# dan64/vs-deoldify

Measured on AMD Instinct MI355X. Metric: colorized frames/sec/GPU @1080p (DeOldify stable rf=35); CIEDE2000 vs ref, higher is better.
Workload: dtype f16

## Files before the change

include/havc_mi355.h:

```cpp
#ifndef HAVC_MI355_H
#define HAVC_MI355_H

#include <stddef.h>
#include <stdint.h>

#ifdef __cplusplus
extern "C" {
#endif

#define HAVC_OK 0
#define HAVC_E_INVALID (-1)
#define HAVC_E_OOM (-2)
#define HAVC_E_HIP (-3)
#define HAVC_E_NODEVICE (-4)
#define HAVC_E_RANGE (-5)

typedef struct havc_ctx havc_ctx;
typedef struct havc_weights havc_weights;
typedef struct havc_net havc_net;

enum havc_op_type {
    HAVC_OP_CONV = 1,
    HAVC_OP_MAXPOOL = 2,
    HAVC_OP_BLUR_RESIZE = 3,
// ... 359 lines not shown
int havc_colormnet_rgb_to_lab(havc_ctx* ctx, const uint8_t* rgb, float* lab, int width, int height);
int havc_colormnet_lab_to_rgb(havc_ctx* ctx, const float* l_plane, const float* ab, uint8_t* rgb, int width, int height);

int havc_cmn_frame_in(havc_ctx* ctx, const uint8_t* rgb, float* lab, float* img, int width, int height, int padded_w, int padded_h, int pad_left,
                      int pad_top);
int havc_cmn_frame_out(havc_ctx* ctx, const float* l_plane, const float* ab_padded, uint8_t* rgb, int width, int height, int padded_w, int padded_h,
                       int pad_left, int pad_top);
int havc_memory_read_banked(havc_ctx* ctx, const float* mk, const float* ms, const float* qk, const float* qe, const float* mv, float* out,
                            float* use_count, float* life_count, int usage_from, int CK, int CV, int N, int64_t pitch, int HW, int top_k);
int havc_memory_read_reserve(havc_ctx* ctx, int N_max, int HW, int top_k);
int havc_cmn_short_term(havc_ctx* ctx, havc_net* net, int first_op, int n_ops, int agg_buf, int short_buf, const float* q, const float* k, const float* v,
                        const float* rel_w, const float* rel_b, float* agg, float* attn, float* short_out, int C, int CV, int H, int W, int max_dis);
int havc_cmn_join_add(havc_ctx* ctx, float* readout, const float* short_out, int64_t n);
int havc_cmn_side_mark(havc_ctx* ctx);
int havc_cmn_side_begin(havc_ctx* ctx);
int havc_cmn_side_end(havc_ctx* ctx);
int havc_cmn_side_wait(havc_ctx* ctx, int apply_usage);
int havc_cmn_value_in(havc_ctx* ctx, const float* image, const float* planes, float* value_in, int64_t pixels);
int havc_dev_copy_2d(havc_ctx* ctx, void* d_dst, size_t dst_pitch, const void* d_src, size_t src_pitch, size_t width_bytes, size_t rows);
int havc_net_bind_many(havc_net* net, int count, const int32_t* bufs, void* const* device_ptrs);
int havc_net_enqueue_slices(havc_net* net, int count, const int32_t* first_op, const int32_t* n_ops, const int32_t* batch);
int havc_debug_stream_jitter(int seed, int max_us);
const char* havc_build_stamp(void);

int havc_tag_timing_enable(havc_ctx* ctx, int tag, int enable);
int havc_tag_timing_read(havc_ctx* ctx, double* avg_ms, int64_t* launches);

#ifdef __cplusplus
}
#endif
#endif
```

vsdeoldify_amd/_native.py:

```python
import ctypes as C
import os

import numpy as np

_HERE = os.path.dirname(os.path.abspath(__file__))
LIB_PATH = os.environ.get("HAVC_MI355_LIB") or os.path.join(_HERE, "lib", "libhavc_mi355.so")

HAVC_OK, HAVC_E_INVALID, HAVC_E_OOM, HAVC_E_HIP, HAVC_E_NODEVICE, HAVC_E_RANGE = 0, -1, -2, -3, -4, -5
RESIZE_SPLINE64, RESIZE_SPLINE36 = 0, 1

OP_CONV, OP_MAXPOOL, OP_BLUR_RESIZE, OP_AFFINE, OP_ATTENTION, OP_PREP_RGB8, OP_COPY_CH = 1, 2, 3, 4, 5, 6, 7
OP_SUBSAMPLE2, OP_PROJ2, OP_BILINEAR2, OP_PREP_LAB_L = 8, 9, 10, 11
OP_DWCONV7, OP_LAYERNORM, OP_MHA, OP_PIXSHUF4_BLUR, OP_PREP_DDCOLOR, OP_DWCONV7_LN = 12, 13, 14, 15, 16, 17
OP_FOLD_QUERIES, OP_SHUF4_BLUR_AB = 18, 19
OP_EW, OP_DWCONV, OP_CHAN_ATTN, OP_MHA64, OP_CBAM, OP_GRU, OP_PLANAR_IN, OP_PLANAR_OUT, OP_CMN_DECODER_IN = 20, 21, 22, 23, 24, 25, 26, 27, 28
OP_SRCREF_ATTN, OP_TSTACK, OP_ELU, OP_PREP_REMASTER, OP_REMASTER_OUT = 29, 30, 31, 32, 33
EW_SRC_BCAST, EW_RES, EW_RES_BCAST, EW_RELU, EW_DUAL = 1, 2, 4, 8, 16
F_RELU_PRE, F_AFFINE, F_RESIDUAL, F_RELU_POST = 0x1, 0x2, 0x4, 0x8
F_OUT_PIXSHUF, F_OUT_TRANSPOSED, F_OUT_RGB8, F_LEAKY, F_FUSE_RGB8, F_PS_BLUR = 0x10, 0x20, 0x40, 0x80, 0x100, 0x200
F_GELU, F_W_FROM_BUF = 0x400, 0x800
F_FUSE_PROJ = 0x2000
F_PRECISE = 0x4000


# ... 214 lines not shown
    ("havc_batcher_create", _I, [_P, _P, _P, _F, _I, _I, _I, C.POINTER(_P)]),
    ("havc_batcher_create_frames", _I, [_P, _I, _P, _I, _I, _I, _I, C.POINTER(_P)]),
    ("havc_batcher_submit", _I, [_P, _P, _P]),
    ("havc_batcher_stats", _I, [_P, C.POINTER(C.c_int64), C.POINTER(C.c_int64)]),
    ("havc_batcher_free", None, [_P]),
    ("havc_cmn_frame_in", _I, [_P, _P, _P, _P, _I, _I, _I, _I, _I, _I]),
    ("havc_cmn_frame_out", _I, [_P, _P, _P, _P, _I, _I, _I, _I, _I, _I]),
    ("havc_memory_read_banked", _I, [_P, _P, _P, _P, _P, _P, _P, _P, _P, _I, _I, _I, _I, C.c_int64, _I, _I]),
    ("havc_memory_read_reserve", _I, [_P, _I, _I, _I]),
    ("havc_cmn_short_term", _I, [_P, _P, _I, _I, _I, _I, _P, _P, _P, _P, _P, _P, _P, _P, _I, _I, _I, _I, _I]),
    ("havc_cmn_join_add", _I, [_P, _P, _P, C.c_int64]),
    ("havc_cmn_side_mark", _I, [_P]),
    ("havc_cmn_side_begin", _I, [_P]),
    ("havc_ctx_set_stream_priority", _I, [_P, _I]),
    ("havc_ctx_set_stream_cus", _I, [_P, _I]),
    ("havc_cmn_side_end", _I, [_P]),
    ("havc_cmn_side_wait", _I, [_P, _I]),
    ("havc_cmn_value_in", _I, [_P, _P, _P, _P, C.c_int64]),
    ("havc_dev_copy_2d", _I, [_P, _P, _SZ, _P, _SZ, _SZ, _SZ]),
    ("havc_net_bind_many", _I, [_P, _I, _P, _P]),
    ("havc_net_enqueue_slices", _I, [_P, _I, _P, _P, _P]),
    ("havc_debug_stream_jitter", _I, [_I, _I]),
    ("havc_build_stamp", C.c_char_p, []),
    ("havc_tag_timing_enable", _I, [_P, _I, _I]),
    ("havc_tag_timing_read", _I, [_P, C.POINTER(C.c_double), C.POINTER(C.c_int64)]),
]


def _preload_torch_hip_runtime():
    if os.environ.get("HAVC_NO_TORCH_HIP_PRELOAD"):
        return
    try:
        import importlib.util
        spec = importlib.util.find_spec("torch")
        if spec is not None and spec.submodule_search_locations:
            p = os.path.join(list(spec.submodule_search_locations)[0], "lib", "libamdhip64.so")
            if os.path.exists(p):
                C.CDLL(p, mode=C.RTLD_GLOBAL)
    except Exception:
        pass


def load():
    global _lib
    if _lib is not None:
        return _lib
# ... 280 lines not shown
```

vsdeoldify_amd/csrc/conv_common.h:

```cpp
#pragma once
#include "kernels.h"
#include "../../include/havc_mi355.h"

typedef _Float16 half8 __attribute__((ext_vector_type(8)));
typedef _Float16 half4 __attribute__((ext_vector_type(4)));
typedef float float4v __attribute__((ext_vector_type(4)));

__device__ __forceinline__ float gelu_erf(float v) {
    const float L2E = 1.44269504088896341f;
    const float v2 = fminf(v * v, 36.0f);
    float p = fmaf(-1.72152684e-05f * -L2E, v2, -5.10199108e-04f * -L2E);
    p = fmaf(p, v2, 7.34616312e-02f * -L2E);
    p = fmaf(p, v2, 1.59538024f * -L2E);
    const float e = __builtin_amdgcn_exp2f(p * v);
    return v * __builtin_amdgcn_rcpf(1.0f + e);
}

__device__ __forceinline__ int64_t out_pixel(const ConvArgs& p, int m, int HoWo) {
    if (p.oss == 1) return m;
    const int b = m / HoWo, rem = m - b * HoWo, ho = rem / p.Wo, wo = rem - ho * p.Wo;
    return ((int64_t)(b * p.Ho * p.oss + ho * p.oss + p.ooy)) * (p.Wo * p.oss) + wo * p.oss + p.oox;
}

__device__ __forceinline__ void split_hl(float v, half_t& hi, half_t& lo) {
    hi = (half_t)v;
    lo = (half_t)((v - (float)hi) * 2048.f);
}
__device__ __forceinline__ float join_hl(half_t hi, half_t lo) { return (float)hi + (float)lo * (1.f / 2048.f); }

__device__ __forceinline__ void epilogue_frag_precise(const ConvArgs& p, const float4v acc, int m, int n, int HoWo) {
    const bool leaky = p.flags & HAVC_F_LEAKY;
    float v[4];
#pragma unroll
    for (int r = 0; r < 4; ++r) v[r] = acc[r] * p.pscale;
    if (p.bias) {
        const float4 bv = *reinterpret_cast<const float4*>(p.bias + n);
        v[0] += bv.x; v[1] += bv.y; v[2] += bv.z; v[3] += bv.w;
    }
    if (p.flags & HAVC_F_OUT_RGB8) {
        if (n == 0) {
            uint8_t* y = reinterpret_cast<uint8_t*>(p.y) + (int64_t)m * 3;
#pragma unroll
            for (int r = 0; r < 3; ++r) {
// ... 149 lines not shown
```

vsdeoldify_amd/csrc/conv_pipe_epilogue.inc:

```
    if (ABL == 5 || ABL == 9 || ABL == 10) {
        float t = 0.f;
#pragma unroll
        for (int mi = 0; mi < FM; ++mi)
#pragma unroll
            for (int ni = 0; ni < FN; ++ni) t += acc[ni][mi][0] + acc[ni][mi][1] + acc[ni][mi][2] + acc[ni][mi][3];
        if (t == 123.456f) reinterpret_cast<half_t*>(p.y)[0] = (half_t)t;
        return;
    }
    constexpr bool PRECISE = (ABL == 30);
    const bool lds_epi = !PRECISE && !(eflags & (HAVC_F_OUT_TRANSPOSED | HAVC_F_OUT_RGB8)) &&
                         (!(eflags & HAVC_F_OUT_PIXSHUF) || (p.Co & 63) == 0);
    bool fused_done = false;
    if (PRECISE && EXTRA && has_extra && (eflags & HAVC_F_FUSE_RGB8)) {
        fused_done = true;
        const bool leaky = eflags & HAVC_F_LEAKY;
        const int rlo = p.res_cpitch >> 1;
        auto fold = [&](const float4v a4, int m, int n, float d[3]) {
            if (n >= p.Npad) return;
            float v[4];
            const float4 bv = p.bias ? *reinterpret_cast<const float4*>(p.bias + n) : make_float4(0.f, 0.f, 0.f, 0.f);
            const float bb[4] = {bv.x, bv.y, bv.z, bv.w};
#pragma unroll
            for (int r = 0; r < 4; ++r) {
                v[r] = a4[r] * p.pscale + bb[r];
// ... 384 lines not shown
#pragma unroll
                for (int w = 0; w < 5; ++w) t += part[(w * BM + pl) * 3 + jo];
                float sg = 1.f / (1.f + __expf(-t));
                sg = sg * (p.f1 - p.f0) + p.f0;
                sg = sg * p.istd[jo] + p.mean[jo];
                sg = fminf(fmaxf(sg, 0.f), 1.f);
                y[jo] = (uint8_t)(int)(sg * 255.f);
            }
        }
    } else if (!EXTRA && (eflags & HAVC_F_FUSE_PROJ) && WM == 2 && WN == 4 && FM == 8) {
        fused_done = true;
        const bool leaky = eflags & HAVC_F_LEAKY;
        const int nw0 = n0 + wn * 64, cw0 = wn * 64;
        float4 bvs[FN];
#pragma unroll
        for (int ni = 0; ni < FN; ++ni)
            bvs[ni] = p.bias ? *reinterpret_cast<const float4*>(p.bias + nw0 + ni * 16 + lg * 4) : make_float4(0.f, 0.f, 0.f, 0.f);
        float4v facc[FM];
        int fb_prev = -1;
        half4 wa[FN];
#pragma unroll
        for (int mi = 0; mi < FM; ++mi) {
            const int mf = gm(wm * (FM * 16) + mi * 16);
            const int fb = mf < p.M ? mf / HoWo : 0;
            if (fb != fb_prev) {
                fb_prev = fb;
#pragma unroll
                for (int ni = 0; ni < FN; ++ni) {
                    wa[ni] = half4{0, 0, 0, 0};
                    if (lr < 2) {
                        const float4 w4 = *reinterpret_cast<const float4*>(p.fuse_w + ((size_t)fb * 2 + lr) * 256 + cw0 + ni * 16 + lg * 4);
                        wa[ni] = half4{(half_t)w4.x, (half_t)w4.y, (half_t)w4.z, (half_t)w4.w};
                    }
                }
            }
            facc[mi] = float4v{0.f, 0.f, 0.f, 0.f};
#pragma unroll
            for (int ni = 0; ni < FN; ++ni) {
                const float bb[4] = {bvs[ni].x, bvs[ni].y, bvs[ni].z, bvs[ni].w};
                half4 o;
#pragma unroll
                for (int r = 0; r < 4; ++r) {
                    float v = acc[ni][mi][r] + bb[r];
                    if (eflags & HAVC_F_RELU_PRE) v = v > 0.f ? v : (leaky ? v * p.f2 : 0.f);
                    o[r] = (half_t)v;
                }
                facc[mi] = __builtin_amdgcn_mfma_f32_16x16x16f16(wa[ni], o, facc[mi], 0, 0, 0);
// ... 38 lines not shown
        char* img = smem + wave * (FM * 2048);
#pragma unroll
        for (int ni = 0; ni < FN; ++ni) {
            const float4 bv = bvA[ni], sc = scA[ni], sh = shA[ni];
            const float bb[4] = {bv.x, bv.y, bv.z, bv.w}, ss[4] = {sc.x, sc.y, sc.z, sc.w}, hh[4] = {sh.x, sh.y, sh.z, sh.w};
#pragma unroll
            for (int mi = 0; mi < FM; ++mi) {
                half4 o;
#pragma unroll
                for (int r = 0; r < 4; ++r) {
                    float v = acc[ni][mi][r] + bb[r];
                    if (eflags & HAVC_F_RELU_PRE) v = v > 0.f ? v : (leaky ? v * p.f2 : 0.f);
                    if (eflags & HAVC_F_GELU) v = gelu_erf(v);
                    if (eflags & HAVC_F_AFFINE) v = v * ss[r] + hh[r];
                    o[r] = (half_t)v;
                }
                const int slot = (ni * 2 + (lg >> 1)) ^ (lp & 7);
                *reinterpret_cast<half4*>(img + mi * 2048 + lp * 128 + slot * 16 + (lg & 1) * 8) = o;
            }
        }
        if ((eflags & HAVC_F_PS_BLUR) && WM == 2 && WN == 4 && FM == 8) {
            __syncthreads();
            const int tile = m0 / BM, tt = p.tiles_y * p.tiles_x;
            const int b = tile / tt, t = tile - b * tt, ty = t / p.tiles_x, tx = t - ty * p.tiles_x;
            const int h0 = ty * 15 - 1, w0 = tx * 15 - 1, H2 = 2 * p.Ho, W2 = 2 * p.Wo;
            half_t* y = reinterpret_cast<half_t*>(p.y) + p.y_coff + (n0 >> 2);
            if (tid < 30 * 2 * 8 && (!p.cstore || (n0 >> 2) + (tid & 7) * 8 < p.cstore)) {
                const int ch = tid & 7, xh = (tid >> 3) & 1, Yl = tid >> 4;
                const int Y = 2 * (h0 + 1) + Yl;
                const int ay0 = max(Y - 1, 0);
                auto ld = [&](int ay, int ax) -> half8 {
                    const int dy = (ay >> 1) - h0, dx = (ax >> 1) - w0, q = (ay & 1) * 2 + (ax & 1);
                    return *reinterpret_cast<const half8*>(smem + ((dy >> 3) * WN + q) * (FM * 2048) + (dy & 7) * 2048 + dx * 128 + ((ch ^ (dx & 7)) << 4));
                };
                if (Y < H2) {
                    const int X0 = 2 * (w0 + 1) + xh * 15;
                    float l0[8], l1[8];
                    {
                        const int axl = max(X0 - 1, 0);
                        const half8 a = ld(ay0, axl), c = ld(Y, axl);
#pragma unroll
                        for (int e = 0; e < 8; ++e) { l0[e] = (float)a[e]; l1[e] = (float)c[e]; }
                    }
                    half_t* yrow = y + ((int64_t)(b * H2 + Y) * W2) * p.y_cpitch + ch * 8;
#pragma unroll 5
                    for (int k = 0; k < 15; ++k) {
                        const int X = X0 + k;
// ... 25 lines not shown
        if (eflags & HAVC_F_RESIDUAL) {
#pragma unroll
            for (int mi = 0; mi < FM; ++mi)
#pragma unroll
                for (int hp = 0; hp < 2; ++hp) {
                    const int m = gm(wm * (FM * 16) + PF(mi) * 16 + (lane >> 3) + hp * 8);
                    rres[mi][hp] = half8{0, 0, 0, 0, 0, 0, 0, 0};
                    if (do_res && m < p.M) rres[mi][hp] = *reinterpret_cast<const half8*>(p.res + opix(m) * p.res_cpitch + p.res_coff + n);
                }
        }
#pragma unroll
        for (int mi = 0; mi < FM; ++mi) {
#pragma unroll
            for (int hp = 0; hp < 2; ++hp) {
                const int px = (lane >> 3) + hp * 8;
                const int m = gm(wm * (FM * 16) + PF(mi) * 16 + px);
                const half8 v = *reinterpret_cast<const half8*>(img + mi * 2048 + px * 128 + ((ch ^ (px & 7)) << 4));
                if (m >= p.M) continue;
                half_t* y = reinterpret_cast<half_t*>(p.y);
                int64_t off;
                if (eflags & HAVC_F_OUT_PIXSHUF) {
                    const int q = n / p.Co, cc = n - q * p.Co;
                    if (q >= 4) continue;
                    const int b = m / HoWo, rem = m - b * HoWo, ho = rem / p.Wo, wo = rem - ho * p.Wo;
                    off = ((int64_t)(b * 2 * p.Ho + 2 * ho + (q >> 1)) * (2 * p.Wo) + 2 * wo + (q & 1)) * p.y_cpitch + p.y_coff + cc;
                } else {
                    if (n >= p.Co) continue;
                    off = opix(m) * p.y_cpitch + p.y_coff + n;
                }
                half8 o = v;
                if (eflags & (HAVC_F_RESIDUAL | HAVC_F_RELU_POST)) {
#pragma unroll
                    for (int e = 0; e < 8; ++e) {
                        float f = (float)v[e];
                        if (eflags & HAVC_F_RESIDUAL) f += (float)rres[mi][hp][e];
                        if (eflags & HAVC_F_RELU_POST) f = f > 0.f ? f : (leaky ? f * p.f2 : 0.f);
                        o[e] = (half_t)f;
                    }
                }
                if (ABL == 12) { if (o[0] == (half_t)123.f && o[1] == (half_t)77.f) *reinterpret_cast<half8*>(y + off) = o; }
                else if (ABL == 14) *reinterpret_cast<half8*>(y + (off & 0xFFFF8)) = o;
                else if (eflags & HAVC_F_NT_STORE) __builtin_nontemporal_store(o, reinterpret_cast<half8*>(y + off));
                else *reinterpret_cast<half8*>(y + off) = o;
            }
        }
    }
    if (EXTRA && has_extra && !(fused_done)) {
#pragma unroll
// ... 6 lines not shown
```

vsdeoldify_amd/csrc/conv_pipe_kernel.inc:

```
namespace {

constexpr int FN = 4;
constexpr unsigned OOB = 0xF0000000u;

template <int WM, int WN, int FM, int EXTRA>
struct Geo {
    static constexpr int NW = WM * WN;
    static constexpr int BM = WM * FM * 16, BN = WN * 64;
    static constexpr int A_IT = BM / 8 / NW, B_IT = BN / 8 / NW;
    static constexpr int NS = 2 * FM;
    static constexpr int PIECES = A_IT + B_IT;
    static constexpr int ROWS = BM + BN + 16 * EXTRA;
    static constexpr int STAGE_BYTES = ROWS * 128;
    static constexpr int LDS_BYTES = 2 * STAGE_BYTES;
    static_assert(BM % (8 * NW) == 0 && BN % (8 * NW) == 0 && NW % 2 == 0, "pieces must divide over an even number of waves");
    static_assert(FM >= FN, "second-half weight fragments are prefetched during the first FM steps");
    static_assert(FM % 2 == 0, "the 4-slot pixel-fragment ring wraps cleanly only when a stage has a multiple of 4 steps");
    static_assert(!EXTRA || (WM == 2 && WN == 4 && FM == 8), "extra columns: 256x256 tile only");
    static_assert(NW * FM * 2048 <= LDS_BYTES, "LDS epilogue image");
};

typedef __attribute__((address_space(3))) void* lds_ptr_t;

__device__ __forceinline__ void dma16(__amdgpu_buffer_rsrc_t rsrc, char* lds_wave_base, unsigned voff, unsigned soff) {
// ... 60 lines not shown
    const int kt0 = SK > 1 ? ((KT * part / SK) & ~1) : 0;
    const int kt1 = SK > 1 ? (part + 1 == SK ? KT : ((KT * (part + 1) / SK) & ~1)) : KT;
    const int2* kt_lane = p.ktab + c;

    unsigned b_voff[B_IT];
#pragma unroll
    for (int it = 0; it < B_IT; ++it) {
        const int n = n0 + (wave + it * NW) * 8 + r8;
        b_voff[it] = n < p.Npad ? (unsigned)((n * p.Kc + c) * 16) : OOB;
    }
    HAVC_STAMP(8);
    int2 e_nx = kt_lane[kt0 * 8];
#pragma unroll
    for (int it = 0; it < B_IT; ++it) dma16(rw, smem + BM * 128 + (wave + it * NW) * 1024, b_voff[it], (unsigned)kt0 * 128u);

    unsigned a_base[A_IT];
    int a_hw0[A_IT];
#pragma unroll
    for (int it = 0; it < A_IT; ++it) {
        const int row = (wave + it * NW) * 8 + r8;
        const int m = m0 + row;
        const bool ok = m < p.M;
        const int mm = ok ? m : 0;
        int b = mm / HoWo;
        const int rem = mm - b * HoWo;
        int ho = rem / p.Wo;
        int wo = rem - ho * p.Wo;
        if ((EF >= 0 ? EF : p.flags) & HAVC_F_PS_BLUR) {
            const int tile = m0 / BM, tt = p.tiles_y * p.tiles_x;
            b = tile / tt;
            const int t = tile - b * tt, ty = t / p.tiles_x, tx = t - ty * p.tiles_x;
            ho = min(max(ty * 15 - 1 + (row >> 4), 0), p.Ho - 1);
            wo = min(max(tx * 15 - 1 + (row & 15), 0), p.Wo - 1);
        }
        const int hi0 = ok ? ho * p.stride - p.pad : -16384, wi0 = wo * p.stride - p.pad_w;
        a_hw0[it] = (hi0 & 0xffff) | (wi0 << 16);
        a_base[it] = (unsigned)((((int64_t)(b * p.Hi + hi0) * p.Wi + wi0) * p.x_cpitch + p.x_coff) * 2);
    }
    const unsigned x_voff = (unsigned)(((n0 + BN + (wave & 1) * 8 + r8) * p.Kc + c) * 16);
    const bool extra_wave = has_extra && wave >= 6;


    auto a_voff = [&](int it, int2 e) -> unsigned {
        const int hi = (short)(a_hw0[it] & 0xffff) + (short)(e.y & 0xffff);
        const int wi = (a_hw0[it] >> 16) + (e.y >> 16);
        const bool ok = ((unsigned)hi < (unsigned)p.Hi) & ((unsigned)wi < (unsigned)p.Wi);
        return ok ? a_base[it] + (unsigned)e.x : OOB;
    };

    const int fsw = (lr >> 1) & 7;
    const int a_l0 = (wm * (FM * 16) + lr) * 128 + ((lg ^ fsw) << 4), a_l1 = a_l0 ^ 64;
    const int b_l0 = BM * 128 + (wn * 64 + lr) * 128 + ((lg ^ fsw) << 4), b_l1 = b_l0 ^ 64;
    const int x_l0 = (BM + BN + lr) * 128 + ((lg ^ fsw) << 4), x_l1 = x_l0 ^ 64;

// ... 15 lines not shown
#pragma unroll
    for (int q = 0; q < A_IT; ++q) dma_piece(q, smem, e_nx, kt0);
    if (EXTRA && extra_wave) dma16(rw, smem + (BM + BN) * 128 + (wave & 1) * 1024, x_voff, 0);
    e_nx = kt_lane[(kt1 - kt0 > 1 ? kt0 + 1 : kt0) * 8];
    if (kt1 - kt0 > 1) {
#pragma unroll
        for (int q = 0; q < EARLY; ++q) dma_piece(q, smem + G::STAGE_BYTES, e_nx, kt0 + 1);
    }
    HAVC_STAMP(9);
    asm volatile("s_waitcnt vmcnt(0)" ::: "memory");
    asm volatile("" : "+v"(e_nx.x), "+v"(e_nx.y));
    __builtin_amdgcn_s_barrier();
    HAVC_STAMP(1);

    half8 bf[2][FN];
    half8 xb[2];
    half8 af[4];
#pragma unroll
    for (int ni = 0; ni < FN; ++ni) bf[0][ni] = *reinterpret_cast<const half8*>(smem + b_l0 + ni * 2048);
    if (EXTRA) xb[0] = *reinterpret_cast<const half8*>(smem + x_l0);
    af[0] = *reinterpret_cast<const half8*>(smem + a_l0 + aoff(0));
    af[1] = *reinterpret_cast<const half8*>(smem + a_l0 + aoff(1));

    auto stage = [&](int kt, auto lvl_tag) {
        constexpr int LVL = ABL == 10 ? 0 : ABL == 1 ? (decltype(lvl_tag)::value ? 1 : 0) : decltype(lvl_tag)::value;
        constexpr bool RD = ABL != 10;
        constexpr bool DMA_ON = ABL != 1;
        const char* cur = smem + (kt & 1) * G::STAGE_BYTES;
        char* nxt = smem + ((kt & 1) ^ 1) * G::STAGE_BYTES;
        int2 e_n2 = e_nx;
#pragma unroll
        for (int s = 0; s < NS; ++s) {
            const int ks = s / FM, mi = s % FM;
            if (s == 0 && LVL == 2) e_n2 = kt_lane[(kt + 2) * 8];
            {
                const int s2 = s + 2;
                if (s2 < NS && RD) af[s2 % 4] = *reinterpret_cast<const half8*>(cur + ((s2 / FM) ? a_l1 : a_l0) + aoff(s2 % FM));
            }
            if (s == NS - 3 && LVL >= 1) {
                asm volatile("s_waitcnt vmcnt(0) lgkmcnt(0)" ::: "memory");
                asm volatile("" : "+v"(e_n2.x), "+v"(e_n2.y));
                __builtin_amdgcn_s_barrier();
            }
            if (s >= NS - 2 && LVL >= 1) {
                const int j = s - (NS - 2);
                af[(s + 2) % 4] = *reinterpret_cast<const half8*>(nxt + a_l0 + aoff(j));
#pragma unroll
                for (int ni = 2 * j; ni < 2 * j + 2; ++ni) bf[0][ni] = *reinterpret_cast<const half8*>(nxt + b_l0 + ni * 2048);
                if (EXTRA && j == 1) xb[0] = *reinterpret_cast<const half8*>(nxt + x_l0);
            }
            if (ks == 0 && mi >= FM - FN && RD)
                bf[1][mi - (FM - FN)] = *reinterpret_cast<const half8*>(cur + b_l1 + (mi - (FM - FN)) * 2048);
            if (EXTRA && s == 3) xb[1] = *reinterpret_cast<const half8*>(cur + x_l1);
            if (LVL >= 1 && DMA_ON && s < NSD) {
#pragma unroll
                for (int q = EARLY + (s * (P - EARLY)) / NSD; q < EARLY + ((s + 1) * (P - EARLY)) / NSD; ++q)
                    dma_piece(q, nxt, e_nx, kt + 1);
            }
            if (EXTRA && LVL >= 1 && DMA_ON && s == NSD) {
                if (extra_wave) dma16(rw, nxt + (BM + BN) * 128 + (wave & 1) * 1024, x_voff, (unsigned)(kt + 1) * 128u);
            }
            if (LVL == 2 && DMA_ON && s >= NS - EARLY)
                dma_piece(s - (NS - EARLY), const_cast<char*>(cur), e_n2, kt + 2);
            const half8 a = af[s % 4];
#pragma unroll
            for (int ni = 0; ni < FN; ++ni) {
                if (ABL == 4 || ABL == 9) asm volatile("" ::"v"(bf[ks][ni]), "v"(a));
                else acc[ni][mi] = __builtin_amdgcn_mfma_f32_16x16x32_f16(bf[ks][ni], a, acc[ni][mi], 0, 0, 0);
            }
            if (EXTRA && mi < 2)
                accx[mi] = __builtin_amdgcn_mfma_f32_16x16x32_f16(xb[ks], a, accx[mi], 0, 0, 0);
            __builtin_amdgcn_sched_barrier(0);
        }
        e_nx = e_n2;
    };
    if (NW == 8 && p.prio && wave >= NW / 2) __builtin_amdgcn_s_setprio(1);
    int kt = kt0;
    for (; kt + 2 < kt1; ++kt) stage(kt, std::integral_constant<int, 2>{});
    if (kt1 - kt0 >= 2) { stage(kt, std::integral_constant<int, 1>{}); ++kt; }
    stage(kt, std::integral_constant<int, 0>{});
    HAVC_STAMP(2);

    auto gm = [&](int local_row) -> int { return m0 + local_row; };
    const int lp = lr;
    if (!EXTRA && SK > 1) {
#pragma unroll
        for (int mi = 0; mi < FM; ++mi) {
            const int m = m0 + wm * (FM * 16) + mi * 16 + lr;
            if (m >= p.M) continue;
            float* row = p.ws + ((int64_t)part * p.M + m) * p.Npad;
#pragma unroll
            for (int ni = 0; ni < FN; ++ni) {
                const int n = n0 + wn * 64 + ni * 16 + lg * 4;
                if (n < p.Npad) *reinterpret_cast<float4v*>(row + n) = acc[ni][mi];
            }
        }
        return;
    }
    const int eflags = EF >= 0 ? (EF | (p.flags & ~HAVC_EPI_MASK)) : p.flags;
    constexpr bool UNIT_STEP = EF >= 0;
    auto opix = [&](int m) -> int64_t { return EF >= 0 ? (int64_t)m : out_pixel(p, m, HoWo); };
#include "conv_pipe_epilogue.inc"
#undef PF
    if (ABL == 40) {
        HAVC_STAMP(5);
        asm volatile("s_waitcnt vmcnt(0)" ::: "memory");
        HAVC_STAMP(6);
        if (tid == 0 && m0 < p.M) {
            unsigned hwid;
            asm volatile("s_getreg_b32 %0, hwreg(HW_REG_HW_ID)" : "=s"(hwid));
            stamps[7] = hwid;
            uint64_t* d = reinterpret_cast<uint64_t*>(reinterpret_cast<half_t*>(p.y) + (int64_t)m0 * p.y_cpitch + p.y_coff + n0);
#pragma unroll
            for (int i = 0; i < 12; ++i) d[i] = stamps[i];
        }
    }
#undef HAVC_STAMP
}

template <auto Kernel>
static void ensure_lds_optin(int lds_bytes) {
    static std::atomic<uint64_t> done{0};
    int dev = 0;
    (void)hipGetDevice(&dev);
// ... 6 lines not shown
```

vsdeoldify_amd/csrc/kernels.h:

```cpp
#pragma once
#include <hip/hip_runtime.h>
#include <stdint.h>

typedef _Float16 half_t;

struct ConvArgs {
    const half_t* x;
    const half_t* w;
    const float* bias;
    const float* scale;
    const float* shift;
    const half_t* res;
    void* y;
    int x_cpitch, x_coff;
    int res_cpitch, res_coff;
    int y_cpitch, y_coff;
    int Hi, Wi, C8;
    int Ho, Wo, Co;
    int kh, kw, stride, pad, dil;
    int pad_w;
    int oss, ooy, oox;
    int Kc, Npad;
    int M;
    int flags;
    int pix_pitch;
    float f0, f1, f2;
    float mean[3], istd[3];
    int cfg;
    const int2* ktab;
    int C8a;
    int tiles_y, tiles_x;
    const float* fuse_w;
    const float* fuse_b;
    uint8_t* fuse_rgb;
    int cstore;
    float* fuse_out;
    unsigned x_bytes;
    unsigned w_bytes;
    int prio;
    int splitk;
    float* ws;
    float pscale;
    int ngroup, rband;
};
inline void conv_raster(ConvArgs& a, int MT, int NT, int BN) {
    static const int on = [] { const char* e = getenv("HAVC_RASTER_GROUP"); return e ? atoi(e) : 0; }();
    a.ngroup = a.rband = 0;
    const double tile_bytes = (double)BN * a.Kc * 16.0;
    if (!on || a.splitk > 1 || NT < 4 || MT < 16 || tile_bytes * NT < 3.5e6) return;
    int ng = (int)(2.5e6 / tile_bytes);
    if (ng < 2 || ng >= NT) return;
    a.ngroup = ng;
    a.rband = (MT + 7) / 8;
}
#define HAVC_KTAB_PAD_DH 0x7fff

int launch_conv(const ConvArgs& a, hipStream_t s);
int launch_conv_pipe(const ConvArgs& a, int cfg, hipStream_t s);
int launch_conv_pipe_ef(const ConvArgs& a, int cfg, hipStream_t s);
bool conv_splitk_cfg_ok(int cfg);
const char* conv_config_name(const ConvArgs& a);

int launch_maxpool3x3s2(const half_t* x, half_t* y, int B, int Hi, int Wi, int Ho, int Wo, int C, int x_cpitch,
                        int x_coff, int y_cpitch, int y_coff, hipStream_t s);
int launch_blur_resize(const half_t* x, half_t* y, int B, int Hi, int Wi, int Ho, int Wo, int C, int x_cpitch,
                       int x_coff, int y_cpitch, int y_coff, hipStream_t s);
// ... 342 lines not shown
```

vsdeoldify_amd/csrc/rt_net.cpp:

```cpp
#include "runtime_internal.h"

namespace {

int run_op(havc_net* n, const havc_op& op, int batch) {
    havc_ctx* c = n->ctx;
    hipStream_t s = c->cur ? c->cur : c->stream;
    int e = 0;
    const bool timed = (op.tag == c->timed_tag && c->timed_tag >= 0 && op.type == HAVC_OP_CONV);
    std::pair<hipEvent_t, hipEvent_t> evp{nullptr, nullptr};
    auto open_tag_pair = [&]() -> int {
        if (c->tag_used == c->tag_events.size()) {
            hipEvent_t a, b;
            HIP_TRY(c, hipEventCreate(&a));
            HIP_TRY(c, hipEventCreate(&b));
            c->tag_events.emplace_back(a, b);
        }
        evp = c->tag_events[c->tag_used++];
        HIP_TRY(c, hipEventRecord(evp.first, s));
        return HAVC_OK;
    };
    if (timed) if (int rc = open_tag_pair()) return rc;
    const bool precise = op.flags & HAVC_F_PRECISE;
    auto fills = [&](int id, uint64_t elems) { return (uint64_t)n->bufdesc[id].elems_per_frame == elems; };
    auto frame_at = [&](int id, int f) { return (char*)bufptr(n, id) + (uint64_t)f * n->bufdesc[id].elems_per_frame * n->bufdesc[id].elem_bytes; };
// ... 50 lines not shown
                    return fail(c, HAVC_E_INVALID, "conv op: FUSE_PROJ buffers: fp32 [2][256] matrix per frame, fp32 [Ho*Wo][Npad/256][2] output");
                a.fuse_w = (const float*)bufptr(n, op.src2);
                a.fuse_out = (float*)bufptr(n, op.aux0);
            }
            a.res = (op.flags & HAVC_F_RESIDUAL) ? (const half_t*)bufptr(n, op.src2) : nullptr;
            a.y = bufptr(n, op.dst);
            a.x_cpitch = op.src_cpitch; a.x_coff = op.src_coff;
            a.res_cpitch = op.res_cpitch; a.res_coff = op.res_coff;
            a.y_cpitch = op.dst_cpitch; a.y_coff = op.dst_coff;
            a.Hi = op.Hi; a.Wi = op.Wi; a.C8 = op.Ci / 8;
            a.Ho = op.Ho; a.Wo = op.Wo; a.Co = op.Co;
            a.kh = op.kh; a.kw = op.kw; a.stride = op.stride; a.pad = op.pad; a.dil = op.dil;
            a.pad_w = op.pad + op.pad_w_delta;
            a.oss = op.out_step == 2 ? 2 : 1; a.ooy = op.out_oy; a.oox = op.out_ox;
            a.Kc = op.Kc; a.Npad = op.Npad;
            a.M = batch * op.Ho * op.Wo;
            a.flags = op.flags;
            if (c->nt_store_bytes && (uint64_t)batch * n->bufdesc[op.dst].elems_per_frame * n->bufdesc[op.dst].elem_bytes >= c->nt_store_bytes)
                a.flags |= HAVC_F_NT_STORE;
            a.pix_pitch = (op.flags & HAVC_F_PS_BLUR) ? 0 : op.aux0;
            a.C8a = (op.aux1 > 0 && op.aux1 < op.Ci / 8) ? op.aux1 : op.Ci / 8;
            a.f0 = op.f0; a.f1 = op.f1; a.f2 = op.f2;
            a.cfg = op.reserved;
            { static const int prio = [] { const char* e = getenv("HAVC_SETPRIO"); return e ? atoi(e) != 0 : 1; }(); a.prio = prio; }
            a.splitk = HAVC_F_SPLITK_COUNT(op.flags);
            if (a.splitk == 1) a.splitk = 0;
            a.pscale = 1.f;
            if (op.flags & HAVC_F_PRECISE) {
                if ((op.flags & HAVC_F_W_FROM_BUF) || a.splitk ||
                    !(op.f3 > 0.f) || (op.src_cpitch & 15) || (!(op.flags & HAVC_F_OUT_RGB8) && (op.dst_cpitch & 15)))
                    return fail(c, HAVC_E_INVALID, "conv op: PRECISE needs a plain conv (no fused / transposed / split-K form), f3 = accumulator scale > 0, hi|lo pixel rows");
                a.pscale = op.f3;
            }
            if (a.splitk) {
                if ((op.flags & (HAVC_F_PS_BLUR | HAVC_F_FUSE_RGB8 | HAVC_F_FUSE_PROJ | HAVC_F_W_FROM_BUF | HAVC_F_OUT_RGB8)) || (op.Kc >> 3) < 2 * a.splitk)
                    return fail(c, HAVC_E_INVALID, "conv op: SPLITK needs a plain conv with at least 2 K stages per part");
                if (s != c->stream && s != c->stream2) return fail(c, HAVC_E_INVALID, "conv op: SPLITK ops run on the ctx's own streams (one workspace per stream)");
                const int slot = s == c->stream ? SCR_SPLITK_MAIN : SCR_SPLITK_SIDE;
                const size_t need = (size_t)a.splitk * batch * op.Ho * op.Wo * op.Npad * 4;
                if (int rc2 = ensure_scratch(c, slot, need)) return rc2;
                a.ws = (float*)c->scratch[slot];
            }
            {
                const int oi = (int)(&op - n->ops.data());
                a.ktab = n->ktab_off[oi] >= 0 ? n->d_ktab + n->ktab_off[oi] : nullptr;
                const uint64_t xb = (uint64_t)n->bufdesc[op.src].elems_per_frame * n->bufdesc[op.src].elem_bytes * n->max_batch + 256;
// ... 484 lines not shown
    if (!c || !blob || !out || nbytes == 0) return fail(c, HAVC_E_INVALID, "weights_load: bad args");
    std::lock_guard<std::mutex> lk(c->mu);
    SetupLock setup;
    HIP_TRY(c, hipSetDevice(c->dev));
    uint8_t* d = nullptr;
    HIP_TRY(c, hipMalloc((void**)&d, nbytes));
    hipError_t e = hipMemcpy(d, blob, nbytes, hipMemcpyHostToDevice);
    if (e != hipSuccess) { (void)hipFree(d); return hip_fail(c, e, "weights H2D"); }
    c->stats.bytes_resident += (int64_t)nbytes;
    *out = new havc_weights{c, d, nbytes};
    return HAVC_OK;
}

void havc_weights_free(havc_weights* w) {
    if (!w) return;
    std::lock_guard<std::mutex> lk(w->ctx->mu);
    SetupLock setup;
    (void)sync_streams(w->ctx);
    (void)hipFree(w->d_blob);
    w->ctx->stats.bytes_resident -= (int64_t)w->nbytes;
    delete w;
}

int havc_net_create(havc_ctx* c, havc_weights* w, const havc_op* ops, int n_ops, const havc_buf* bufs, int n_bufs,
                    int in_buf, int out_buf, int S, int max_batch, havc_net** out) {
    if (!c || !w || !ops || !bufs || !out || n_ops <= 0 || n_bufs <= 0 || max_batch < 1)
        return fail(c, HAVC_E_INVALID, "net_create: bad args");
    if (in_buf < 0 || in_buf >= n_bufs || out_buf < 0 || out_buf >= n_bufs) return fail(c, HAVC_E_INVALID, "net_create: in/out buffer id");
    std::lock_guard<std::mutex> lk(c->mu);
    SetupLock setup;
    HIP_TRY(c, hipSetDevice(c->dev));
    for (int i = 0; i < n_ops; ++i) {
        const havc_op& o = ops[i];
        auto bad = [&](int id) { return id < -1 || id >= n_bufs; };
        if (bad(o.src) || bad(o.src2) || bad(o.dst) || o.src < 0 || o.dst < 0) return fail(c, HAVC_E_INVALID, "net_create: op buffer id out of range");
        if (o.type == HAVC_OP_ATTENTION && (o.aux1 < 0 || o.aux1 >= n_bufs)) return fail(c, HAVC_E_INVALID, "net_create: attention V^T buffer id");
        if (o.type == HAVC_OP_CONV && (o.flags & (HAVC_F_RESIDUAL | HAVC_F_W_FROM_BUF)) && o.src2 < 0)
            return fail(c, HAVC_E_INVALID, "net_create: conv op with RESIDUAL / W_FROM_BUF needs a buffer in src2");
        for (int64_t off : {o.w_off, o.bias_off, o.scale_off, o.shift_off})
            if (off >= 0 && ((size_t)off >= w->nbytes || (off & 15))) return fail(c, HAVC_E_INVALID, "net_create: weight offset out of range / unaligned");
    }
    havc_net* n = new havc_net();
    n->ctx = c; n->w = w;
    n->ops.assign(ops, ops + n_ops);
    n->bufdesc.assign(bufs, bufs + n_bufs);
    n->bufs.assign(n_bufs, nullptr);
    n->in_buf = in_buf; n->out_buf = out_buf; n->S = S; n->max_batch = max_batch;
    for (int i = 0; i < n_ops; ++i) n->flops_per_frame += (double)ops[i].flops;
    for (int i = 0; i < n_ops; ++i)
        if (ops[i].tag == 1) { n->tail_first = i; break; }
    size_t ktab_bytes = 0;
    {
        std::vector<int2> host;
        n->ktab_off.assign(n_ops, -1);
        for (int i = 0; i < n_ops; ++i) {
            const havc_op& o = ops[i];
            if (o.type != HAVC_OP_CONV) continue;
            n->ktab_off[i] = (int64_t)host.size();
            const int C8 = o.Ci / 8, C8a = (o.aux1 > 0 && o.aux1 < C8) ? o.aux1 : C8;
            const size_t start = host.size();
            auto emit = [&](int kh, int kw, int c) {
                int2 e;
                e.x = ((kh * o.dil * o.Wi + kw * o.dil) * o.src_cpitch + c * 8) * 2;
                e.y = (int)(((unsigned)(kh * o.dil) & 0xffffu) | ((unsigned)(kw * o.dil) << 16));
                host.push_back(e);
            };
            auto emit_seg = [&](int c_lo, int c_hi) {
                if (c_hi <= c_lo) return;
                if (c_lo == 0 && c_hi % 8 == 0) {
                    for (int g = 0; g < c_hi / 8; ++g)
                        for (int kh = 0; kh < o.kh; ++kh)
                            for (int kw = 0; kw < o.kw; ++kw)
                                for (int c = 0; c < 8; ++c) emit(kh, kw, g * 8 + c);
                } else {
                    for (int kh = 0; kh < o.kh; ++kh)
                        for (int kw = 0; kw < o.kw; ++kw)
                            for (int c = c_lo; c < c_hi; ++c) emit(kh, kw, c);
                }
                while ((host.size() - start) % 8) host.push_back(int2{0, HAVC_KTAB_PAD_DH});
            };
            emit_seg(0, C8a);
            emit_seg(C8a, C8);
            if (o.flags & HAVC_F_PRECISE) {
                const size_t len = host.size() - start;
                for (int rep = 1; rep < 3; ++rep)
                    for (size_t k = 0; k < len; ++k) {
                        int2 e = host[start + k];
                        if (rep == 2 && (short)(e.y & 0xffff) != HAVC_KTAB_PAD_DH) e.x += o.src_cpitch;
                        host.push_back(e);
                    }
            }
            if ((int)(host.size() - start) != o.Kc) {
                delete n;
                return fail(c, HAVC_E_INVALID, "net_create: conv op Kc does not match its K layout (Ci, kh, kw, aux1)");
            }
        }
        if (!host.empty()) {
            hipError_t e = hipMalloc((void**)&n->d_ktab, host.size() * sizeof(int2));
            if (e == hipSuccess) e = hipMemcpy(n->d_ktab, host.data(), host.size() * sizeof(int2), hipMemcpyHostToDevice);
            if (e != hipSuccess) {
                if (n->d_ktab) (void)hipFree(n->d_ktab);
                delete n;
                return hip_fail(c, e, "K table upload");
            }
            ktab_bytes = host.size() * sizeof(int2);
            c->stats.bytes_resident += (int64_t)ktab_bytes;
        }
    }
    for (int i = 0; i < n_bufs; ++i) {
        size_t nb = (size_t)bufs[i].elems_per_frame * bufs[i].elem_bytes * max_batch + 256;
        hipError_t e = hipMalloc(&n->bufs[i], nb);
        if (e == hipSuccess && (bufs[i].zero_init || c->range_check)) e = hipMemset(n->bufs[i], 0, nb);
        if (e != hipSuccess) {
            for (int k = 0; k <= i; ++k) {
                if (!n->bufs[k]) continue;
                (void)hipFree(n->bufs[k]);
                if (k < i) c->stats.bytes_resident -= (int64_t)((size_t)bufs[k].elems_per_frame * bufs[k].elem_bytes * max_batch + 256);
            }
// ... 253 lines not shown
```

vsdeoldify_amd/csrc/runtime_internal.h:

```cpp
#pragma once
#include "../../include/havc_mi355.h"
#include "kernels.h"

#include <algorithm>
#include <atomic>
#include <cmath>
#include <cstdio>
#include <cstdlib>
#include <cstring>
#include <map>
#include <mutex>
#include <string>
#include <tuple>
#include <vector>

extern std::recursive_mutex g_setup_mu;
struct SetupLock {
    bool on;
    SetupLock() {
        static const bool enabled = [] { const char* e = getenv("HAVC_SETUP_MUTEX"); return e ? atoi(e) != 0 : true; }();
        on = enabled;
        if (on) g_setup_mu.lock();
    }
    ~SetupLock() { if (on) g_setup_mu.unlock(); }
// ... 93 lines not shown
    int timed_tag = -1;
    std::vector<std::pair<hipEvent_t, hipEvent_t>> tag_events;
    size_t tag_used = 0;
    double tag_ms = 0;
    int64_t tag_launches = 0;
};

struct havc_weights {
    havc_ctx* ctx;
    uint8_t* d_blob;
    size_t nbytes;
};

struct havc_net {
    havc_ctx* ctx;
    havc_weights* w;
    std::vector<havc_op> ops;
    std::vector<havc_buf> bufdesc;
    std::vector<void*> bufs;
    int in_buf, out_buf, S, max_batch;
    int tail_first = -1;
    int2* d_ktab = nullptr;
    std::vector<int64_t> ktab_off;
    const void* in_override = nullptr;
    void* out_override = nullptr;
    unsigned* d_range = nullptr;
    bool range_ready = false;
    std::vector<float> range_absmax;
    std::vector<int64_t> range_bad;
    std::vector<void*> bound;
    double flops_per_frame = 0;
};

inline int fail(havc_ctx* c, int code, const std::string& msg) {
    if (c) c->err = msg; else g_create_error = msg;
    return code;
}

inline int hip_fail(havc_ctx* c, hipError_t e, const char* what) {
    std::string m = std::string(what) + ": " + hipGetErrorString(e);
    (void)hipGetLastError();
    return fail(c, e == hipErrorOutOfMemory ? HAVC_E_OOM : HAVC_E_HIP, m);
}

#define HIP_TRY(ctx, expr)                                         \
    do {                                                           \
// ... 184 lines not shown
```

Measured before the change: 360.7.

## Use magic-number division for conv indexing and skip empty final K half-step

Replaces integer divisions by Ho*Wo, Wo and tile counts in the conv pipeline kernel and epilogue with precomputed multiply-shift divisors set per op on the host. It also detects at net creation when the last K group's upper half is entirely padding, and in the final pipeline stage skips the second half of MFMA steps in that case. The aim is to cut integer ALU cost in address computation and to avoid wasted MFMAs on padded K entries. It adds per-op host setup and a test-only helper export, and relies on the fast-division being exact across the dividend range and on the skip check matching the stage's step layout.

```diff
diff --git a/include/havc_mi355.h b/include/havc_mi355.h
--- a/include/havc_mi355.h
+++ b/include/havc_mi355.h
@@ -405,6 +405,7 @@
 int havc_net_enqueue_slices(havc_net* net, int count, const int32_t* first_op, const int32_t* n_ops, const int32_t* batch);
 int havc_debug_stream_jitter(int seed, int max_us);
 const char* havc_build_stamp(void);
+int havc_conv_fast_div(uint32_t divisor, const uint32_t* dividends, uint32_t* quotients, int64_t count);
 
 int havc_tag_timing_enable(havc_ctx* ctx, int tag, int enable);
 int havc_tag_timing_read(havc_ctx* ctx, double* avg_ms, int64_t* launches);
diff --git a/vsdeoldify_amd/_native.py b/vsdeoldify_amd/_native.py
--- a/vsdeoldify_amd/_native.py
+++ b/vsdeoldify_amd/_native.py
@@ -260,6 +260,7 @@
     ("havc_net_enqueue_slices", _I, [_P, _I, _P, _P, _P]),
     ("havc_debug_stream_jitter", _I, [_I, _I]),
     ("havc_build_stamp", C.c_char_p, []),
+    ("havc_conv_fast_div", _I, [C.c_uint32, _P, _P, C.c_int64]),
     ("havc_tag_timing_enable", _I, [_P, _I, _I]),
     ("havc_tag_timing_read", _I, [_P, C.POINTER(C.c_double), C.POINTER(C.c_int64)]),
 ]
diff --git a/vsdeoldify_amd/csrc/conv_common.h b/vsdeoldify_amd/csrc/conv_common.h
--- a/vsdeoldify_amd/csrc/conv_common.h
+++ b/vsdeoldify_amd/csrc/conv_common.h
@@ -1,6 +1,7 @@
 #pragma once
 #include "kernels.h"
 #include "../../include/havc_mi355.h"
+#include <algorithm>
 
 typedef _Float16 half8 __attribute__((ext_vector_type(8)));
 typedef _Float16 half4 __attribute__((ext_vector_type(4)));
@@ -16,9 +17,28 @@
     return v * __builtin_amdgcn_rcpf(1.0f + e);
 }
 
+__host__ __device__ __forceinline__ unsigned fast_div(unsigned n, const FastDiv d) {
+    return d.mul ? (unsigned)(((uint64_t)n * d.mul) >> 32) >> d.sh : n;
+}
+inline FastDiv fast_div_make(unsigned d) {
+    if (d <= 1) return FastDiv{0u, 0u};
+    unsigned l = 0;
+    while ((1ull << l) < d) ++l;
+    const uint64_t pw = 1ull << (31 + l);
+    return FastDiv{(unsigned)((pw + d - 1) / d), l - 1};
+}
+inline void conv_set_divisors(ConvArgs& a) {
+    a.fd_howo = fast_div_make((unsigned)std::max(a.Ho * a.Wo, 1));
+    a.fd_wo = fast_div_make((unsigned)std::max(a.Wo, 1));
+    a.fd_tt = fast_div_make((unsigned)std::max(a.tiles_y * a.tiles_x, 1));
+    a.fd_tx = fast_div_make((unsigned)std::max(a.tiles_x, 1));
+}
+
+template <bool FD = false>
 __device__ __forceinline__ int64_t out_pixel(const ConvArgs& p, int m, int HoWo) {
     if (p.oss == 1) return m;
-    const int b = m / HoWo, rem = m - b * HoWo, ho = rem / p.Wo, wo = rem - ho * p.Wo;
+    const int b = FD ? (int)fast_div((unsigned)m, p.fd_howo) : m / HoWo, rem = m - b * HoWo;
+    const int ho = FD ? (int)fast_div((unsigned)rem, p.fd_wo) : rem / p.Wo, wo = rem - ho * p.Wo;
     return ((int64_t)(b * p.Ho * p.oss + ho * p.oss + p.ooy)) * (p.Wo * p.oss) + wo * p.oss + p.oox;
 }
 
diff --git a/vsdeoldify_amd/csrc/conv_pipe_epilogue.inc b/vsdeoldify_amd/csrc/conv_pipe_epilogue.inc
--- a/vsdeoldify_amd/csrc/conv_pipe_epilogue.inc
+++ b/vsdeoldify_amd/csrc/conv_pipe_epilogue.inc
@@ -430,7 +430,7 @@
 #pragma unroll
         for (int mi = 0; mi < FM; ++mi) {
             const int mf = gm(wm * (FM * 16) + mi * 16);
-            const int fb = mf < p.M ? mf / HoWo : 0;
+            const int fb = mf < p.M ? (int)fast_div((unsigned)mf, p.fd_howo) : 0;
             if (fb != fb_prev) {
                 fb_prev = fb;
 #pragma unroll
@@ -515,7 +515,7 @@
         if ((eflags & HAVC_F_PS_BLUR) && WM == 2 && WN == 4 && FM == 8) {
             __syncthreads();
             const int tile = m0 / BM, tt = p.tiles_y * p.tiles_x;
-            const int b = tile / tt, t = tile - b * tt, ty = t / p.tiles_x, tx = t - ty * p.tiles_x;
+            const int b = (int)fast_div((unsigned)tile, p.fd_tt), t = tile - b * tt, ty = (int)fast_div((unsigned)t, p.fd_tx), tx = t - ty * p.tiles_x;
             const int h0 = ty * 15 - 1, w0 = tx * 15 - 1, H2 = 2 * p.Ho, W2 = 2 * p.Wo;
             half_t* y = reinterpret_cast<half_t*>(p.y) + p.y_coff + (n0 >> 2);
             if (tid < 30 * 2 * 8 && (!p.cstore || (n0 >> 2) + (tid & 7) * 8 < p.cstore)) {
@@ -587,8 +587,8 @@
                 if (eflags & HAVC_F_OUT_PIXSHUF) {
                     const int q = n / p.Co, cc = n - q * p.Co;
                     if (q >= 4) continue;
-                    const int b = m / HoWo, rem = m - b * HoWo, ho = rem / p.Wo, wo = rem - ho * p.Wo;
-                    off = ((int64_t)(b * 2 * p.Ho + 2 * ho + (q >> 1)) * (2 * p.Wo) + 2 * wo + (q & 1)) * p.y_cpitch + p.y_coff + cc;
+                    const int b = (int)fast_div((unsigned)m, p.fd_howo), rem = m - b * HoWo, ho = (int)fast_div((unsigned)rem, p.fd_wo), wo = rem - ho * p.Wo;
+                    off =((int64_t)(b * 2 * p.Ho + 2 * ho + (q >> 1)) * (2 * p.Wo) + 2 * wo + (q & 1)) * p.y_cpitch + p.y_coff + cc;
                 } else {
                     if (n >= p.Co) continue;
                     off = opix(m) * p.y_cpitch + p.y_coff + n;
diff --git a/vsdeoldify_amd/csrc/conv_pipe_kernel.inc b/vsdeoldify_amd/csrc/conv_pipe_kernel.inc
--- a/vsdeoldify_amd/csrc/conv_pipe_kernel.inc
+++ b/vsdeoldify_amd/csrc/conv_pipe_kernel.inc
@@ -106,14 +106,14 @@
         const int m = m0 + row;
         const bool ok = m < p.M;
         const int mm = ok ? m : 0;
-        int b = mm / HoWo;
+        int b = (int)fast_div((unsigned)mm, p.fd_howo);
         const int rem = mm - b * HoWo;
-        int ho = rem / p.Wo;
+        int ho = (int)fast_div((unsigned)rem, p.fd_wo);
         int wo = rem - ho * p.Wo;
         if ((EF >= 0 ? EF : p.flags) & HAVC_F_PS_BLUR) {
             const int tile = m0 / BM, tt = p.tiles_y * p.tiles_x;
-            b = tile / tt;
-            const int t = tile - b * tt, ty = t / p.tiles_x, tx = t - ty * p.tiles_x;
+            b = (int)fast_div((unsigned)tile, p.fd_tt);
+            const int t = tile - b * tt, ty = (int)fast_div((unsigned)t, p.fd_tx), tx = t - ty * p.tiles_x;
             ho = min(max(ty * 15 - 1 + (row >> 4), 0), p.Ho - 1);
             wo = min(max(tx * 15 - 1 + (row & 15), 0), p.Wo - 1);
         }
@@ -175,15 +175,15 @@
     af[0] = *reinterpret_cast<const half8*>(smem + a_l0 + aoff(0));
     af[1] = *reinterpret_cast<const half8*>(smem + a_l0 + aoff(1));
 
-    auto stage = [&](int kt, auto lvl_tag) {
+    auto stage = [&](int kt, auto lvl_tag, const bool skip2) {
         constexpr int LVL = ABL == 10 ? 0 : ABL == 1 ? (decltype(lvl_tag)::value ? 1 : 0) : decltype(lvl_tag)::value;
+        constexpr bool MAY_SKIP = decltype(lvl_tag)::value == 0 && ABL != 30;
         constexpr bool RD = ABL != 10;
         constexpr bool DMA_ON = ABL != 1;
         const char* cur = smem + (kt & 1) * G::STAGE_BYTES;
         char* nxt = smem + ((kt & 1) ^ 1) * G::STAGE_BYTES;
         int2 e_n2 = e_nx;
-#pragma unroll
-        for (int s = 0; s < NS; ++s) {
+        auto step = [&](const int s) __attribute__((always_inline)) {
             const int ks = s / FM, mi = s % FM;
             if (s == 0 && LVL == 2) e_n2 = kt_lane[(kt + 2) * 8];
             {
@@ -224,14 +224,20 @@
             if (EXTRA && mi < 2)
                 accx[mi] = __builtin_amdgcn_mfma_f32_16x16x32_f16(xb[ks], a, accx[mi], 0, 0, 0);
             __builtin_amdgcn_sched_barrier(0);
+        };
+#pragma unroll
+        for (int s = 0; s < FM; ++s) step(s);
+        if (!(MAY_SKIP && skip2)) {
+#pragma unroll
+            for (int s = FM; s < NS; ++s) step(s);
         }
         e_nx = e_n2;
     };
     if (NW == 8 && p.prio && wave >= NW / 2) __builtin_amdgcn_s_setprio(1);
     int kt = kt0;
-    for (; kt + 2 < kt1; ++kt) stage(kt, std::integral_constant<int, 2>{});
-    if (kt1 - kt0 >= 2) { stage(kt, std::integral_constant<int, 1>{}); ++kt; }
-    stage(kt, std::integral_constant<int, 0>{});
+    for (; kt + 2 < kt1; ++kt) stage(kt, std::integral_constant<int, 2>{}, false);
+    if (kt1 - kt0 >= 2) { stage(kt, std::integral_constant<int, 1>{}, false); ++kt; }
+    stage(kt, std::integral_constant<int, 0>{}, p.k_half_empty && kt1 == KT);
     HAVC_STAMP(2);
 
     auto gm = [&](int local_row) -> int { return m0 + local_row; };
@@ -252,7 +258,7 @@
     }
     const int eflags = EF >= 0 ? (EF | (p.flags & ~HAVC_EPI_MASK)) : p.flags;
     constexpr bool UNIT_STEP = EF >= 0;
-    auto opix = [&](int m) -> int64_t { return EF >= 0 ? (int64_t)m : out_pixel(p, m, HoWo); };
+    auto opix = [&](int m) -> int64_t { return EF >= 0 ? (int64_t)m : out_pixel<ABL != 30>(p, m, HoWo); };
 #include "conv_pipe_epilogue.inc"
 #undef PF
     if (ABL == 40) {
diff --git a/vsdeoldify_amd/csrc/kernels.h b/vsdeoldify_amd/csrc/kernels.h
--- a/vsdeoldify_amd/csrc/kernels.h
+++ b/vsdeoldify_amd/csrc/kernels.h
@@ -3,6 +3,8 @@
 #include <stdint.h>
 
 typedef _Float16 half_t;
+
+struct FastDiv { unsigned mul, sh; };
 
 struct ConvArgs {
     const half_t* x;
@@ -42,6 +44,9 @@
     float* ws;
     float pscale;
     int ngroup, rband;
+    FastDiv fd_howo, fd_wo;
+    FastDiv fd_tt, fd_tx;
+    int k_half_empty;
 };
 inline void conv_raster(ConvArgs& a, int MT, int NT, int BN) {
     static const int on = [] { const char* e = getenv("HAVC_RASTER_GROUP"); return e ? atoi(e) : 0; }();
diff --git a/vsdeoldify_amd/csrc/rt_net.cpp b/vsdeoldify_amd/csrc/rt_net.cpp
--- a/vsdeoldify_amd/csrc/rt_net.cpp
+++ b/vsdeoldify_amd/csrc/rt_net.cpp
@@ -1,4 +1,5 @@
 #include "runtime_internal.h"
+#include "conv_common.h"
 
 namespace {
 
@@ -96,6 +97,8 @@
             a.C8a = (op.aux1 > 0 && op.aux1 < op.Ci / 8) ? op.aux1 : op.Ci / 8;
             a.f0 = op.f0; a.f1 = op.f1; a.f2 = op.f2;
             a.cfg = op.reserved;
+            conv_set_divisors(a);
+            a.k_half_empty = n->k_half_empty[(size_t)(&op - n->ops.data())];
             { static const int prio = [] { const char* e = getenv("HAVC_SETPRIO"); return e ? atoi(e) != 0 : 1; }(); a.prio = prio; }
             a.splitk = HAVC_F_SPLITK_COUNT(op.flags);
             if (a.splitk == 1) a.splitk = 0;
@@ -626,6 +629,13 @@
     delete w;
 }
 
+int havc_conv_fast_div(uint32_t divisor, const uint32_t* dividends, uint32_t* quotients, int64_t count) {
+    if (divisor < 1 || divisor > 0x80000000u || count < 0 || (count > 0 && (!dividends || !quotients))) return HAVC_E_INVALID;
+    const FastDiv fd = fast_div_make(divisor);
+    for (int64_t i = 0; i < count; ++i) quotients[i] = fast_div(dividends[i], fd);
+    return HAVC_OK;
+}
+
 int havc_net_create(havc_ctx* c, havc_weights* w, const havc_op* ops, int n_ops, const havc_buf* bufs, int n_bufs,
                     int in_buf, int out_buf, int S, int max_batch, havc_net** out) {
     if (!c || !w || !ops || !bufs || !out || n_ops <= 0 || n_bufs <= 0 || max_batch < 1)
@@ -657,6 +667,7 @@
     {
         std::vector<int2> host;
         n->ktab_off.assign(n_ops, -1);
+        n->k_half_empty.assign(n_ops, 0);
         for (int i = 0; i < n_ops; ++i) {
             const havc_op& o = ops[i];
             if (o.type != HAVC_OP_CONV) continue;
@@ -698,6 +709,11 @@
                 delete n;
                 return fail(c, HAVC_E_INVALID, "net_create: conv op Kc does not match its K layout (Ci, kh, kw, aux1)");
             }
+            if (o.Kc >= 8 && !(o.Kc & 7) && !(o.flags & (HAVC_F_PRECISE | HAVC_F_W_FROM_BUF))) {
+                bool empty = true;
+                for (int k = 4; k < 8; ++k) empty = empty && (short)(host[start + o.Kc - 8 + k].y & 0xffff) == HAVC_KTAB_PAD_DH;
+                n->k_half_empty[i] = empty;
+            }
         }
         if (!host.empty()) {
             hipError_t e = hipMalloc((void**)&n->d_ktab, host.size() * sizeof(int2));
diff --git a/vsdeoldify_amd/csrc/runtime_internal.h b/vsdeoldify_amd/csrc/runtime_internal.h
--- a/vsdeoldify_amd/csrc/runtime_internal.h
+++ b/vsdeoldify_amd/csrc/runtime_internal.h
@@ -139,6 +139,7 @@
     int tail_first = -1;
     int2* d_ktab = nullptr;
     std::vector<int64_t> ktab_off;
+    std::vector<uint8_t> k_half_empty;
     const void* in_override = nullptr;
     void* out_override = nullptr;
     unsigned* d_range = nullptr;
```

Result: faster. 364.8, median of 6 (+1.1%).
